# ishine/minimax-speech

Measured on AMD Instinct MI355X. Metric: 24 kHz audio-seconds generated per wall-second per node (CosyVoice2-0.5B-shaped LM + flow + DAC-VAE, end to end), higher is better.
Workload: dtype bf16

## Files before the change

### include/mmx_hip.h

```cpp
#ifndef MMX_HIP_H
#define MMX_HIP_H
#include <stdint.h>
#ifdef __cplusplus
extern "C" {
#endif

#ifndef __HIP__
typedef struct ihipStream_t* hipStream_t;
#endif

#define MMX_F32 0
#define MMX_BF16 1
#define MMX_X2 2
#define MMX_X3 3
#define MMX_X2W 0x12
#define MMX_X3W 0x13
#define MMX_H2 4
#define MMX_H2W 0x14

#define MMX_ACT_NONE 0
#define MMX_ACT_LRELU 1
#define MMX_ACT_GELU 2
#define MMX_ACT_SILU 3
#define MMX_ACT_MISH 4
#define MMX_ACT_TANH 5

int mmx_abi_version(void);

typedef struct MmxGemmParams {
    const void* A;
    const void* W;
    const float* bias;
    const float* residual;
    const float* rowmask;
    const float* alpha;
    float* out_f32;
    void* out_act;
    int64_t lda, ldw, ldr, ldo_f, ldo_a;
    int64_t a_bstride, w_bstride, r_bstride, rm_bstride, of_bstride, oa_bstride;
    int64_t row_off, row_lo, row_hi;
    int64_t out_off, out_len;
    int32_t M, N, batch;
    int32_t ntaps, cin, dil;
    int32_t bias_mod, alpha_mod, bias_per_row;
    int32_t act, act2;
    float slope;
    int32_t row_stride;
} MmxGemmParams;
int mmx_gemm_win(const MmxGemmParams* p, int dtype, hipStream_t stream);
#define MMX_TILE_128x128 1
#define MMX_TILE_128x64 2
#define MMX_TILE_64x64 3
#define MMX_TILE_32x64 4
int mmx_gemm_win_tile(const MmxGemmParams* p, int dtype, int tile, hipStream_t stream);

int mmx_rownorm(const float* x, int64_t ldx, int64_t x_bstride, int rows, int C, int batch,
                const float* gamma, const float* beta, float eps, int rms, int act,
                const float* rowmask, int64_t rm_bstride, const float* addvec, int64_t av_bstride,
                float* out_f32, int64_t ldo_f, int64_t of_bstride,
                void* out_act, int64_t ldo_a, int64_t oa_bstride, int dtype, hipStream_t stream);

int mmx_groupnorm(const float* x, int B, int T, int C, int groups, const float* gamma, const float* beta, float eps,
                  int act, const float* rowmask, void* out, int dtype, hipStream_t stream);

int mmx_act_rows(const float* x, int64_t rows, int C, int act, const float* rowmask, float* out_f32, void* out_act, int dtype,
                 hipStream_t stream);

int mmx_gather_rows(const int64_t* ids, int n, const float* table, int C, float scale, const float* rowmask,
                    float* out_f32, int64_t ldo_f, void* out_act, int64_t ldo_a, int dtype, hipStream_t stream);

int mmx_copy2d(const void* in, int in_dtype, int64_t ibs, int64_t irs, int64_t ics, int rep,
               void* out, int out_dtype, int64_t obs, int64_t ors, int64_t ocs,
               int rows, int cols, int batch, hipStream_t stream);

int mmx_est_pack(const float* x, int64_t x_bs, int x_mod, const float* mu, const float* spks, const float* cond, int B, int T, int C,
                 void* h, int64_t ldh, int dtype, hipStream_t stream);
int mmx_sinusoidal_emb(const float* t, int B, int dim, float scale, void* out, int dtype, hipStream_t stream);

int mmx_cfg_euler(float* x, const float* d_cond, const float* d_uncond, float cfg, float dt, int64_t n,
                  hipStream_t stream);

int mmx_attn_dense(const void* q, int64_t ldq, int64_t q_bs, const void* k, int64_t ldk, int64_t k_bs,
                   const void* v, int64_t ldv, int64_t v_bs, void* out, int64_t ldo, int64_t o_bs,
                   int B, int H, int D, int Tq, int Tk, float scale, const float* keymask, int64_t km_bs, int chunk,
                   const void* pos, int64_t ldp, const float* pos_u, const float* pos_v,
                   int head_stride, int q_begin, int dtype, hipStream_t stream);
int mmx_attn_flash_bf16(const void* q, int64_t ldq, int64_t q_bs, const void* k, int64_t ldk, int64_t k_bs,
                        const void* vt, int64_t ldvt, int64_t vt_bs, void* out, int64_t ldo, int64_t o_bs,
                        int B, int H, int T, float scale, const float* keymask, int64_t km_bs, int chunk, int q_begin,
                        const int32_t* klen, hipStream_t stream);
int mmx_attn_relpos_x(const float* q, int64_t ldq, int64_t q_bs, const float* k, int64_t ldk, int64_t k_bs, const float* v,
                      int64_t ldv, int64_t v_bs, const float* pos, int64_t ldp, const float* pos_u, const float* pos_v,
                      float* out, int64_t ldo, int64_t o_bs, int B, int H, int T, float scale, int chunk, const int32_t* klen,
                      hipStream_t stream);
int mmx_attn_flash_x(const float* q, int64_t ldq, int64_t q_bs, const float* k, int64_t ldk, int64_t k_bs,
                     const float* v, int64_t ldv, int64_t v_bs, float* out, int64_t ldo, int64_t o_bs,
                     int B, int H, int T, float scale, const float* keymask, int64_t km_bs, int chunk,
                     int q_begin, const int32_t* klen, hipStream_t stream);
int mmx_attn_flash_xs(const void* qk, int64_t ldqk, int64_t qk_bs, const void* vt, int64_t ldvt, int64_t vt_bs,
                      float* out, int64_t ldo, int64_t o_bs, int B, int H, int T, float scale, const float* keymask,
                      int64_t km_bs, int chunk, int q_begin, const int32_t* klen, int form, hipStream_t stream);
int mmx_attn_relpos_bf16(const void* q, int64_t ldq, int64_t q_bs, const void* k, int64_t ldk, int64_t k_bs,
                         const void* vt, int64_t ldvt, int64_t vt_bs, const void* pos, int64_t ldp,
                         const float* pos_u, const float* pos_v, void* out, int64_t ldo, int64_t o_bs,
                         int B, int H, int T, float scale, int chunk, const int32_t* klen, hipStream_t stream);

int mmx_attn_flash_fp8(const void* q, int64_t ldq, int64_t q_bs, const void* k, int64_t ldk, int64_t k_bs,
                       const void* vt, int64_t ldvt, int64_t vt_bs, void* out, int64_t ldo, int64_t o_bs,
                       int B, int H, int T, float scale, const float* keymask, int64_t km_bs, int chunk, int q_begin,
                       const int32_t* klen, hipStream_t stream);

int mmx_conv_cin1(const float* x, int64_t x_bs, int T, int C, int k, const float* w, const float* bias, float slope,
                  const float* alpha, float* out_f32, void* out_act, int batch, int dtype, hipStream_t stream);
int mmx_vae_sample(const float* ml, const float* noise, int64_t rows, int D, float* z, float* m, float* logs,
                   hipStream_t stream);
int mmx_mask_rows(void* x, int64_t rows, int C, const float* rowmask, int dtype, hipStream_t stream);
int mmx_pool_rows(const float* x, int64_t x_bs, int rows, int C, int batch, const float* mask, int64_t m_bs, void* out,
                  int64_t ldo, int dtype, hipStream_t stream);
int mmx_prefetch4(const void* p0, int64_t n0, const void* p1, int64_t n1, const void* p2, int64_t n2, const void* p3, int64_t n3,
                  void* sink, int workgroups, hipStream_t stream);
int mmx_resample_linear(const float* x, int64_t rows, int T, int T2, float* out, hipStream_t stream);

int mmx_conv_cout1_tanh(const void* act, int64_t a_bs, int T, int C, int k, const float* w, const float* bias,
                        float slope, int use_tanh, float* out, int64_t o_bs, int batch, int dtype, hipStream_t stream);

#define MMX_X_PACKED 1
#define MMX_OUT_PACKED 2
int mmx_pack_skinny(const void* w, int64_t ldw, int N, int K, const float* kscale, int interleave_half,
                    void* wp, int dtype, hipStream_t stream);
int mmx_skinny_gemm(const void* x, int x_dtype, int64_t ldx, int B, int K, int N, const void* wp,
                    const float* bias, int rs, float eps, int epi, float* out_f32, int64_t ldo_f,
                    void* out_act, int64_t ldo_a, int dtype, int flags, const float* kgamma, hipStream_t stream);

int mmx_decode_prep(const float* x, int64_t ldx, int B, int K, const float* gamma, float* h, int64_t ldh, void* xs,
                    float* ssq, int dtype, hipStream_t stream);
int mmx_skinny2(const void* xs, int B, int K, int N, const void* wp, const float* bias, const float* ssq_in, float eps,
                int epi, float* out, int64_t ldo, void* xs_out, const float* gamma_next, float* ssq_out,
                int tiles_per_wg, int ksplit, float* part, int64_t part_floats, int32_t* tickets, int dtype,
                hipStream_t stream);

int mmx_rope_kv_store(const float* qkv, int64_t ldqkv, int64_t qkv_bs, int B, int rows, int Hq, int Hkv, int D,
                      const float* inv_freq, const int32_t* pos, void* q_out, int64_t ldq, int64_t q_bs,
                      void* kc, void* vc, const int32_t* block_table, int max_pages, int page,
                      int dtype, hipStream_t stream);
int mmx_paged_attn(const void* q, int64_t ldq, int64_t q_bs, int B, int rows, int Hq, int Hkv, int D, float scale,
                   const int32_t* pos, const void* kc, const void* vc, const int32_t* block_table, int max_pages,
                   int page, void* out, int64_t ldo, int64_t o_bs, int dtype, hipStream_t stream);
#define MMX_DA_PACKED 1
#define MMX_DA_PER_HEAD 2
#define MMX_DA_SPLIT 4
#define MMX_DA_H2 8
#define MMX_DA_ONE_HEAD 16
int mmx_decode_attn(const float* qkv, int64_t ldqkv, int B, int Hq, int Hkv, int D, const float* inv_freq,
                    const float* rope_tab, const int32_t* pos, void* kc, void* vc, const int32_t* block_table, int max_pages, int page,
                    float scale, void* out, int64_t ldo, int dtype, int out_packed, hipStream_t stream);
int mmx_decode_attn_fin(const float* qkv, int64_t ldqkv, int B, int Hq, int Hkv, int D, const float* inv_freq,
                        const float* rope_tab, const int32_t* pos, const int32_t* finished, void* kc, void* vc,
                        const int32_t* block_table, int max_pages, int page, float scale, void* out, int64_t ldo, int dtype,
                        int out_packed, hipStream_t stream);
int mmx_swiglu(const float* gu, int64_t ldgu, int rows, int I, void* out, int64_t ldo, int dtype, hipStream_t stream);

int mmx_sample_step(const float* logits, int64_t ldl, int V, int B, int eos_id, int top_k, float top_p,
                    int win_size, float tau_r, uint64_t seed, int32_t* state, int32_t* out_tokens, int max_out,
                    int32_t* sampled, const int32_t* forced, const float* speech_emb, int E, float* next_x,
                    int64_t ldx, float* logp_out, hipStream_t stream);
int mmx_sample_step_tab(const float* logits, int64_t ldl, int V, int B, int eos_id, const int32_t* samp, int32_t* state,
                        int32_t* out_tokens, int max_out, int32_t* sampled, const int32_t* forced, const float* speech_emb,
                        int E, float* next_x, int64_t ldx, float* logp_out, hipStream_t stream);

typedef struct MmxEstNext {
    const void* wqkv;
    const float* n1g;
    const float* n1b;
    void* q_out;
    void* vt_out;
    int64_t q_bs, vt_bs;
    int32_t ldq, ldvt;
} MmxEstNext;
typedef struct MmxEstTailParams {
    const void* ao;
    float* x;
    const void* wo;
    const void* w1;
    const void* w2;
    const float* bo;
    const float* b1;
    const float* b2;
    const float* n3g;
    const float* n3b;
    const float* rowmask;
    void* act_out;
    int64_t ao_bs, x_bs, rm_bs, act_bs;
    int32_t ldao, act_ld, B, T;
    int32_t t_begin;
    float eps;
    MmxEstNext next;
} MmxEstTailParams;
typedef struct MmxEstResnetParams {
    const void* a_in;
    float* x;
    const void* w1;
    const void* w2;
    const void* wr;
    const float* b1;
    const float* g1;
    const float* be1;
    const float* b2;
    const float* g2;
    const float* be2;
    const float* br;
    const float* tv;
    const float* rowmask;
    int64_t a_bs, x_bs, tv_bs, rm_bs;
    int32_t lda, cin, B, T;
    int32_t t_begin;
    float eps;
    MmxEstNext next;
} MmxEstResnetParams;
int mmx_est_tail(const MmxEstTailParams* p, int dtype, int bm, int cfg, hipStream_t stream);
int mmx_est_resnet(const MmxEstResnetParams* p, int dtype, int bm, int cfg, hipStream_t stream);
typedef struct {
    const float* x;
    float* x_out;
    void* act_out;
    const void* w7;
    const void* w1;
    const float* b7;
    const float* b1;
    const float* a0;
    const float* a2;
    const float* alpha_next;
    const int32_t* lens;
    int64_t x_bs;
    int32_t B, T, C, dil;
    float slope;
} MmxDacRuParams;
int mmx_dac_ru(const MmxDacRuParams* p, int dtype, int bm, hipStream_t stream);

int mmx_logmel(const float* wave, int64_t w_bs, int L, int B, const float* gain, const int32_t* lens, const int32_t* h_lens,
               const void* basis, const void* filt, int n_fft, int hop, int bin0, int n_bins, int n_mels, float* out_cm,
               int64_t ldo, void* out_tm, int T, int dtype, hipStream_t stream);

int mmx_logmel_w(const float* wave, int64_t w_bs, int L, int B, const int32_t* lens, const int32_t* h_lens, const void* basis,
                 const void* filt, int n_fft, int hop, int bin0, int n_bins, int n_mels, float* out_cm, int64_t ldo,
                 void* out_tm, int T, int dtype, hipStream_t stream);

int mmx_s3_rope_fsmn(float* qkv, int64_t ldqkv, int64_t qkv_bs, int B, int T, int C, const float* x, int64_t x_bs, float* r,
                     int64_t r_bs, const float* wt, const float* rope_cos, const float* rope_sin, int rope_rows,
                     const int32_t* lens, hipStream_t stream);

int mmx_fsq_encode(const float* x, int64_t ldx, int64_t x_bs, int B, int T, int C, const float* W, const float* bias,
                   const int32_t* lens, int32_t* ids, int64_t ld_ids, float* pre, hipStream_t stream);

#define MMX_RESAMPLE_NOUT 1024
int mmx_resample_sinc(const float* wave, int64_t w_bs, int L, int B, const int32_t* lens, const int32_t* h_lens, int orig, int neu,
                      int width, const float* taps, const int32_t* first, const int32_t* count, int cmax, float* out,
                      int64_t o_bs, int out_cols, hipStream_t stream);

#define MMX_LOUD_PAD 0
#define MMX_LOUD_DROP 1
#define MMX_LOUD_MAX_CH 5
int mmx_kweight_blocks(const float* wave, int64_t w_bs, int L, int B, const int32_t* lens, int rate, int partial, const double* tab,
                       int seg, double* work, int cap, double* energy, int64_t e_bs, float* peak, hipStream_t stream);
int mmx_loudness_gate(const double* energy, int64_t e_bs, int cap, const float* peak, const int32_t* lens, int L, int nclips, int nch,
                      const double* G, int rate, int partial, float* lufs, int want_gain, float target_db, float max_peak, float* gain,
                      uint8_t* mask, int64_t mask_bs, hipStream_t stream);
int mmx_scale_rows(const float* x, int64_t x_bs, int L, int B, const int32_t* lens, const float* gain, int nch, float* out,
                   int64_t o_bs, hipStream_t stream);

int mmx_spec_dist(const float* x, int64_t x_bs, const float* y, int64_t y_bs, int L, int B, const int32_t* lens, const int32_t* h_lens,
                  const void* basis, const void* filt, int n_fft, int n_mels, double eps, double pow, double* work, int cap,
                  double* out, hipStream_t stream);
int mmx_wave_sums(const float* x, int64_t x_bs, const float* y, int64_t y_bs, int L, int B, const int32_t* lens, float clip, double* work,
                  int cap, double* out, hipStream_t stream);

int mmx_gate_threshold(const float* x, int64_t x_bs, int L, int B, const int32_t* lens, const int32_t* h_lens, const void* basis,
                       int n_fft, double n_std, double* work, int cap, float* thresh, int64_t t_bs, hipStream_t stream);
int mmx_gate_analyze(const float* x, int64_t x_bs, int L, int B, const int32_t* lens, const int32_t* h_lens, const void* basis, int n_fft,
                     const float* thresh, int64_t t_bs, float* spec, uint8_t* mask, int frames_cap, hipStream_t stream);
int mmx_gate_synthesize(const float* spec, const uint8_t* mask, int frames_cap, int L, int B, const int32_t* lens, const int32_t* h_lens,
                        const void* inv, const float* window, int n_fft, int n_freq, int n_time, const float* amount, float* frames,
                        float* out, int64_t o_bs, hipStream_t stream);

int mmx_stoi_select(const float* ref, int64_t r_bs, int L, int B, const int32_t* lens, const int32_t* h_lens, const float* window,
                    double* energy, uint8_t* mask, int32_t* map, int32_t* kept, int cap, hipStream_t stream);
int mmx_stoi_bands(const float* est, int64_t e_bs, const float* ref, int64_t r_bs, int L, int B, const int32_t* lens,
                   const int32_t* h_lens, const float* window, const int32_t* map, const int32_t* kept, const void* basis,
                   const void* filt, float* env, int cap, hipStream_t stream);
int mmx_stoi_score(const float* env, int cap, int B, const int32_t* kept, int extended, double* work, int wcap, double* out,
                   int32_t* frames, hipStream_t stream);

int mmx_ir_prepare(const float* ir, int64_t ir_bs, int Lir, int B, const int32_t* ir_lens, const int32_t* h_ir_lens, int Lsig,
                   const int32_t* sig_lens, const int32_t* h_sig_lens, const float* drr, int t0, const double* hann, int start_at_max,
                   float* h_out, int64_t h_bs, int32_t* p, float* s, int32_t* taps, float* drr_out, void* table, int kcap,
                   hipStream_t stream);
int mmx_fir_rows(const float* x, int64_t x_bs, int L, int B, const int32_t* lens, const int32_t* h_lens, const void* table, int kcap,
                 const int32_t* p, const float* s, const int32_t* taps, int wrap, float* out, int64_t o_bs, float* peak,
                 hipStream_t stream);
int mmx_row_absmax(const float* x, int64_t x_bs, int L, int B, const int32_t* lens, float* peak, hipStream_t stream);
int mmx_mix_rows(const float* x, int64_t x_bs, int L, int B, const int32_t* lens, const float* noise, int64_t n_bs, int Ln,
                 const int32_t* nlens, const float* lx, const float* ln, const float* snr, float* out, int64_t o_bs, hipStream_t stream);

#ifdef __cplusplus
}
#endif
#endif
```

### minimax-speech_amd/csrc/gemm.hip

```cpp
#include <algorithm>
#include "common.h"
#include "gemm.h"
#include <utility>

template <typename T> struct Frag;
template <> struct Frag<bf16_t> {
    static constexpr int CH = 8;
    static constexpr int LDS_ROW = 48;
};
template <> struct Frag<float> {
    static constexpr int CH = 4;
    static constexpr int LDS_ROW = 40;
};

template <typename T, typename TA, int NS, int BM, int BN, int WM, int WN, int NWP = 1>
__global__ __launch_bounds__(256) void gemm_win_kernel(GemmParams p) {
    constexpr int BK = 32;
    constexpr bool XS = NS > 1;
    static_assert(NWP == 1 || NWP == NS, "weight planes: as many as activation planes");
    static_assert(!XS || (sizeof(T) == 2 && sizeof(TA) == 4), "split build: bf16 weights, fp32 activations");
    static_assert(XS || sizeof(T) == sizeof(TA), "one storage type otherwise");
    constexpr int CH = Frag<T>::CH;
    constexpr int CPR = BK / CH;
    constexpr int CHA = 16 / sizeof(TA);
    constexpr int CPRA = BK / CHA;
    constexpr int LR = Frag<T>::LDS_ROW;
    constexpr int MF = BM / WM / 16, NF = BN / WN / 16;
    constexpr int A_CHUNKS = (BM * CPRA + 255) / 256, W_CHUNKS = (BN * CPR + 255) / 256;
    constexpr bool A_FULL = (BM * CPRA) % 256 == 0, W_FULL = (BN * CPR) % 256 == 0;
    constexpr bool PRECISE = sizeof(TA) == 4;

    extern __shared__ __attribute__((aligned(16))) char smem[];
    T* As = reinterpret_cast<T*>(smem);
    T* Ws = As + NS * 2 * BM * LR;

    const int tid = threadIdx.x, lane = tid & 63, wave = tid >> 6;
    const int wm = wave / WN, wn = wave % WN;
    const int g = lane >> 4, l16 = lane & 15;
    const int b = blockIdx.z;
    const int m0 = blockIdx.y * BM, n0 = blockIdx.x * BN;

    const TA* A = reinterpret_cast<const TA*>(p.A) + (long)b * p.a_bstride;
    const T* W = reinterpret_cast<const T*>(p.W) + (long)b * p.w_bstride;

    constexpr unsigned OOB = 0x80000000u;
    const auto a_rsrc = __builtin_amdgcn_make_buffer_rsrc(const_cast<TA*>(A), 0, 0x7fffffff, 0x00020000);
    const auto w_rsrc = __builtin_amdgcn_make_buffer_rsrc(const_cast<T*>(W), 0, 0x7fffffff, 0x00020000);
    unsigned a_off[A_CHUNKS];
    int a_c[A_CHUNKS], a_tap[A_CHUNKS];
    long a_srow[A_CHUNKS];
    bool a_mok[A_CHUNKS];
    const unsigned tap_jump = (unsigned)(((long)p.dil * p.lda - p.cin) * (long)sizeof(TA));
#pragma unroll
    for (int i = 0; i < A_CHUNKS; ++i) {
        const int id = tid + i * 256;
        const int r = id / CPRA, k = (id % CPRA) * CHA;
        const int m = m0 + r;
        a_tap[i] = k / p.cin;
        a_c[i] = k % p.cin;
        a_srow[i] = (long)m * p.row_stride + (long)a_tap[i] * p.dil + p.row_off;
        a_off[i] = (unsigned)((a_srow[i] * p.lda + a_c[i]) * (long)sizeof(TA));
        a_mok[i] = (m < p.M) && (A_FULL || id < BM * CPRA);
    }
    unsigned w_off[W_CHUNKS];
#pragma unroll
    for (int i = 0; i < W_CHUNKS; ++i) {
        const int id = tid + i * 256;
        const int r = id / CPR, kc = (id % CPR) * CH;
        const int n = n0 + r;
        const bool ok = (n < p.N) && (W_FULL || id < BN * CPR);
        w_off[i] = ok ? (unsigned)(((long)n * p.ldw + kc) * (long)sizeof(T)) : OOB;
    }
    constexpr int STAGES = (sizeof(T) == 2 && !XS) ? 4 : 2;
    uint4 a_reg[STAGES][A_CHUNKS], w_reg[STAGES][NWP][W_CHUNKS];
    const unsigned w_plane = (unsigned)((p.ldw / NWP) * (long)sizeof(T));
    const int K = p.ntaps * p.cin;
    const int nk = (K + BK - 1) / BK;

    auto load_tile = [&](int kt, auto slot_c) {
        constexpr int slot = decltype(slot_c)::value;
        typedef __attribute__((ext_vector_type(4))) unsigned int u32x4_t;
#pragma unroll
        for (int i = 0; i < A_CHUNKS; ++i) {
            const bool ok = a_mok[i] && (a_tap[i] < p.ntaps) && (a_srow[i] >= p.row_lo) && (a_srow[i] < p.row_hi);
            const u32x4_t v = __builtin_amdgcn_raw_buffer_load_b128(a_rsrc, ok ? a_off[i] : OOB, 0, 0);
            a_reg[slot][i] = make_uint4(v[0], v[1], v[2], v[3]);
            a_off[i] += BK * (unsigned)sizeof(TA);
            a_c[i] += BK;
            while (a_c[i] >= p.cin) {
                a_c[i] -= p.cin;
                a_tap[i]++;
                a_srow[i] += p.dil;
                a_off[i] += tap_jump;
            }
        }
#pragma unroll
        for (int i = 0; i < W_CHUNKS; ++i) {
#pragma unroll
            for (int p2 = 0; p2 < NWP; ++p2) {
                const u32x4_t v = __builtin_amdgcn_raw_buffer_load_b128(w_rsrc, (kt < nk && w_off[i] != OOB) ? w_off[i] + p2 * w_plane : OOB, 0, 0);
                w_reg[slot][p2][i] = make_uint4(v[0], v[1], v[2], v[3]);
            }
            if (w_off[i] != OOB) w_off[i] += BK * (unsigned)sizeof(T);
        }
    };
    auto store_tile = [&](int stage, auto slot_c) {
        constexpr int slot = decltype(slot_c)::value;
#pragma unroll
        for (int i = 0; i < A_CHUNKS; ++i) {
            int id = tid + i * 256;
            if (A_FULL || id < BM * CPRA) {
                if constexpr (XS) {
                    const uint4 v = a_reg[slot][i];
                    float x[4] = {__uint_as_float(v.x), __uint_as_float(v.y), __uint_as_float(v.z), __uint_as_float(v.w)};
#pragma unroll
                    for (int s2 = 0; s2 < NS; ++s2) {
                        uint2 pk;
                        pk.x = pack_bf16x2(x[0], x[1]);
                        pk.y = pack_bf16x2(x[2], x[3]);
                        *reinterpret_cast<uint2*>(As + ((s2 * 2 + stage) * BM + id / CPRA) * LR + (id % CPRA) * CHA) = pk;
                        if (s2 + 1 < NS) {
                            x[0] -= __uint_as_float(pk.x << 16); x[1] -= __uint_as_float(pk.x & 0xffff0000u);
                            x[2] -= __uint_as_float(pk.y << 16); x[3] -= __uint_as_float(pk.y & 0xffff0000u);
                        }
                    }
                } else {
                    *reinterpret_cast<uint4*>(As + (stage * BM + id / CPRA) * LR + (id % CPRA) * CHA) = a_reg[slot][i];
                }
            }
        }
#pragma unroll
        for (int i = 0; i < W_CHUNKS; ++i) {
            int id = tid + i * 256;
            if (W_FULL || id < BN * CPR) {
#pragma unroll
                for (int p2 = 0; p2 < NWP; ++p2)
                    *reinterpret_cast<uint4*>(Ws + ((p2 * 2 + stage) * BN + id / CPR) * LR + (id % CPR) * CH) = w_reg[slot][p2][i];
            }
        }
    };

    float4_t acc[MF][NF];
#pragma unroll
    for (int i = 0; i < MF; ++i)
#pragma unroll
        for (int j = 0; j < NF; ++j) acc[i][j] = float4_t{0.f, 0.f, 0.f, 0.f};

    auto compute = [&](int st) {
        const T* as = As + (st * BM + wm * (BM / WM) + l16) * LR;
        const T* ws = Ws + (st * BN + wn * (BN / WN) + l16) * LR;
        if constexpr (sizeof(T) == 2) {
            short8_t bfr[NWP][NF];
#pragma unroll
            for (int p2 = 0; p2 < NWP; ++p2)
#pragma unroll
                for (int j = 0; j < NF; ++j) bfr[p2][j] = *reinterpret_cast<const short8_t*>(ws + p2 * 2 * BN * LR + j * 16 * LR + 8 * g);
#pragma unroll
            for (int s2 = 0; s2 < NS; ++s2) {
                short8_t af[MF];
#pragma unroll
                for (int i = 0; i < MF; ++i) af[i] = *reinterpret_cast<const short8_t*>(as + s2 * 2 * BM * LR + i * 16 * LR + 8 * g);
#pragma unroll
                for (int p2 = 0; p2 < NWP; ++p2) {
                    if (s2 + p2 >= NS) continue;
#pragma unroll
                    for (int i = 0; i < MF; ++i)
#pragma unroll
                        for (int j = 0; j < NF; ++j)
                            acc[i][j] = __builtin_amdgcn_mfma_f32_16x16x32_bf16(af[i], bfr[p2][j], acc[i][j], 0, 0, 0);
                }
            }
        } else {
#pragma unroll
            for (int c = 0; c < 2; ++c) {
                float4_t af[MF], bfr[NF];
#pragma unroll
                for (int i = 0; i < MF; ++i) af[i] = *reinterpret_cast<const float4_t*>(as + i * 16 * LR + 16 * c + 4 * g);
#pragma unroll
                for (int j = 0; j < NF; ++j) bfr[j] = *reinterpret_cast<const float4_t*>(ws + j * 16 * LR + 16 * c + 4 * g);
#pragma unroll
                for (int s = 0; s < 4; ++s)
#pragma unroll
                    for (int i = 0; i < MF; ++i)
#pragma unroll
                        for (int j = 0; j < NF; ++j)
                            acc[i][j] = __builtin_amdgcn_mfma_f32_16x16x4f32(af[i][s], bfr[j][s], acc[i][j], 0, 0, 0);
            }
        }
    };
    auto for_each_slot = [&](auto&& fn) {
        [&]<int... S>(std::integer_sequence<int, S...>) { (fn(std::integral_constant<int, S>{}), ...); }
        (std::make_integer_sequence<int, STAGES>{});
    };
    for_each_slot([&](auto sc) { load_tile(decltype(sc)::value, sc); });
    int kt0 = 0;
    for (; kt0 + STAGES <= nk; kt0 += STAGES) {
        for_each_slot([&](auto sc) {
            const int kt = kt0 + decltype(sc)::value;
            store_tile(decltype(sc)::value & 1, sc);
            load_tile(kt + STAGES, sc);
            __syncthreads();
            compute(decltype(sc)::value & 1);
        });
    }
    for_each_slot([&](auto sc) {
        const int kt = kt0 + decltype(sc)::value;
        if (kt < nk) {
            store_tile(decltype(sc)::value & 1, sc);
            __syncthreads();
            compute(decltype(sc)::value & 1);
        }
    });

    __syncthreads();
    constexpr int WNC = BN / WN;
    constexpr int CW = WNC / 4;
    constexpr int LDC = WNC + 4;
    float* Cs = reinterpret_cast<float*>(smem) + wave * 16 * LDC;
    float* outf = p.out_f32 ? p.out_f32 + (long)b * p.of_bstride : nullptr;
    TA* outa = p.out_act ? reinterpret_cast<TA*>(p.out_act) + (long)b * p.oa_bstride : nullptr;
    const float* res = p.residual ? p.residual + (long)b * p.r_bstride : nullptr;
    const float* rmask = p.rowmask ? p.rowmask + (long)b * p.rm_bstride : nullptr;
    constexpr int VA = 16 / sizeof(TA);
    const bool vec_f = outf && (p.ldo_f % 4 == 0) && (p.out_off % 4 == 0) && (p.of_bstride % 4 == 0) && ((uintptr_t)p.out_f32 % 16 == 0);
    const bool vec_a = outa && (p.ldo_a % VA == 0) && (p.out_off % VA == 0) && (p.oa_bstride % VA == 0) && ((uintptr_t)p.out_act % 16 == 0) && (CW % VA == 0);
    const bool vec_r = res && (p.ldr % 4 == 0) && (p.r_bstride % 4 == 0) && ((uintptr_t)p.residual % 16 == 0);
    const int erow = lane >> 2, ecol = (lane & 3) * CW;
    auto epilogue = [&](auto act_k, auto act2_k) {
    constexpr int ACT = decltype(act_k)::value, ACT2 = decltype(act2_k)::value;
#pragma unroll
    for (int i = 0; i < MF; ++i) {
#pragma unroll
        for (int j = 0; j < NF; ++j)
#pragma unroll
            for (int r = 0; r < 4; ++r) Cs[(4 * g + r) * LDC + j * 16 + l16] = acc[i][j][r];
        __builtin_amdgcn_fence(__ATOMIC_RELEASE, "wavefront");
        __builtin_amdgcn_wave_barrier();
        float v[CW];
#pragma unroll
        for (int c = 0; c < CW; c += 4) {
            float4_t t4 = *reinterpret_cast<const float4_t*>(Cs + erow * LDC + ecol + c);
            v[c] = t4[0]; v[c + 1] = t4[1]; v[c + 2] = t4[2]; v[c + 3] = t4[3];
        }
        __builtin_amdgcn_wave_barrier();
        const int m = m0 + wm * (BM / WM) + i * 16 + erow;
        const int nb = n0 + wn * WNC + ecol;
        if (m >= p.M || nb >= p.N) continue;
        const bool full = nb + CW <= p.N;
        const float rm = rmask ? rmask[m] : 1.f;
        float rr[CW];
        if (res) {
            if (vec_r && full) {
#pragma unroll
                for (int c = 0; c < CW; c += 4) {
                    float4_t t4 = *reinterpret_cast<const float4_t*>(res + (long)m * p.ldr + nb + c);
                    rr[c] = t4[0]; rr[c + 1] = t4[1]; rr[c + 2] = t4[2]; rr[c + 3] = t4[3];
                }
            } else {
#pragma unroll
                for (int c = 0; c < CW; ++c) rr[c] = (nb + c < p.N) ? res[(long)m * p.ldr + nb + c] : 0.f;
            }
        }
        int bidx = p.bias ? (p.bias_per_row ? m : nb % p.bias_mod) : 0;
        int aidx = p.alpha ? nb % p.alpha_mod : 0;
        float w2[CW];
#pragma unroll
        for (int c = 0; c < CW; ++c) {
            float x = v[c];
            if (p.bias) {
                x += p.bias[bidx];
                if (!p.bias_per_row && ++bidx == p.bias_mod) bidx = 0;
            }
            x = act_c<ACT, PRECISE>(x, p.slope);
            if (res) x += rr[c];
            x *= rm;
            v[c] = x;
            if (outa) {
                float w = act_c<ACT2, PRECISE>(x, p.slope);
                if (p.alpha) {
                    w = snake_apply<PRECISE>(w, p.alpha[aidx]);
                    if (++aidx == p.alpha_mod) aidx = 0;
                }
                w2[c] = w;
            }
        }
        if (outf) {
            const long lin = (long)m * p.ldo_f + nb + p.out_off;
            if (vec_f && full && lin >= 0 && lin + CW <= p.out_len) {
#pragma unroll
                for (int c = 0; c < CW; c += 4)
                    *reinterpret_cast<float4_t*>(outf + lin + c) = float4_t{v[c], v[c + 1], v[c + 2], v[c + 3]};
            } else {
#pragma unroll
                for (int c = 0; c < CW; ++c)
                    if (nb + c < p.N && lin + c >= 0 && lin + c < p.out_len) outf[lin + c] = v[c];
            }
        }
        if (outa) {
            const long lin = (long)m * p.ldo_a + nb + p.out_off;
            if (vec_a && full && lin >= 0 && lin + CW <= p.out_len) {
                if constexpr (sizeof(TA) == 2) {
#pragma unroll
                    for (int c = 0; c < CW; c += 8) {
                        uint4 pk;
                        pk.x = pack_bf16x2(w2[c], w2[c + 1]);
                        pk.y = pack_bf16x2(w2[c + 2], w2[c + 3]);
                        pk.z = pack_bf16x2(w2[c + 4], w2[c + 5]);
                        pk.w = pack_bf16x2(w2[c + 6], w2[c + 7]);
                        *reinterpret_cast<uint4*>(outa + lin + c) = pk;
                    }
                } else {
#pragma unroll
                    for (int c = 0; c < CW; c += 4)
                        *reinterpret_cast<float4_t*>(outa + lin + c) = float4_t{w2[c], w2[c + 1], w2[c + 2], w2[c + 3]};
                }
            } else {
#pragma unroll
                for (int c = 0; c < CW; ++c)
                    if (nb + c < p.N && lin + c >= 0 && lin + c < p.out_len) outa[lin + c] = Cvt<TA>::from_f(w2[c]);
            }
        }
    }
    };
    using std::integral_constant;
    switch (p.act) {
        case ACT_LRELU: epilogue(integral_constant<int, ACT_LRELU>{}, integral_constant<int, ACT_NONE>{}); break;
        case ACT_GELU: epilogue(integral_constant<int, ACT_GELU>{}, integral_constant<int, ACT_NONE>{}); break;
        case ACT_SILU: epilogue(integral_constant<int, ACT_SILU>{}, integral_constant<int, ACT_NONE>{}); break;
        case ACT_MISH: epilogue(integral_constant<int, ACT_MISH>{}, integral_constant<int, ACT_NONE>{}); break;
        case ACT_TANH: epilogue(integral_constant<int, ACT_TANH>{}, integral_constant<int, ACT_NONE>{}); break;
        default:
            if (p.act2 == ACT_MISH) epilogue(integral_constant<int, ACT_NONE>{}, integral_constant<int, ACT_MISH>{});
            else epilogue(integral_constant<int, ACT_NONE>{}, integral_constant<int, ACT_NONE>{});
    }
}

template <typename T, typename TA, int NS, int BM, int BN, int WM, int WN, int NWP = 1>
static int launch_cfg(const GemmParams& p, hipStream_t s) {
    dim3 grid((p.N + BN - 1) / BN, (p.M + BM - 1) / BM, p.batch);
    size_t lds = (size_t)2 * (NS * BM + NWP * BN) * Frag<T>::LDS_ROW * sizeof(T);
    const size_t lds_epi = (size_t)4 * 16 * (BN / WN + 4) * sizeof(float);
    if (lds_epi > lds) lds = lds_epi;
    MMX_LDS_OPT_IN((gemm_win_kernel<T, TA, NS, BM, BN, WM, WN, NWP>), lds);
    hipLaunchKernelGGL((gemm_win_kernel<T, TA, NS, BM, BN, WM, WN, NWP>), grid, dim3(256), lds, s, p);
    MMX_LAUNCH_CHECK();
    return MMX_OK;
}

template <typename T, typename TA, int NS, int NWP = 1>
static int launch_T(const GemmParams& p, hipStream_t s, int force_tile) {
    constexpr int CH = Frag<T>::CH;
    constexpr int CHA = 16 / sizeof(TA);
    MMX_CHECK_ARG(p.A && p.W && p.M > 0 && p.N > 0 && p.batch > 0 && p.ntaps >= 1);
    MMX_CHECK_ARG(p.cin % CH == 0 && p.lda % CHA == 0 && p.ldw % CH == 0);
    MMX_CHECK_ARG(p.a_bstride % CHA == 0 && p.w_bstride % CH == 0);
    MMX_CHECK_ARG(p.ldw % NWP == 0 && (p.ldw / NWP) % CH == 0 && p.ldw / NWP >= ((p.ntaps * p.cin + 31) / 32) * 32);
    MMX_CHECK_ARG(p.bias_mod > 0 && p.alpha_mod > 0 && p.row_stride >= 1);
    MMX_CHECK_ARG(((uintptr_t)p.A % 16) == 0 && ((uintptr_t)p.W % 16) == 0);
    MMX_CHECK_ARG(p.out_f32 || p.out_act);
    const long a_rows = std::min<long>(p.row_hi, (long)(p.M - 1) * p.row_stride + (long)(p.ntaps - 1) * p.dil + p.row_off + 1);
    MMX_CHECK_ARG((double)a_rows * (double)p.lda * sizeof(TA) < 2147483000.0 &&
                  (double)p.N * (double)p.ldw * sizeof(T) < 2147483000.0);
    MMX_CHECK_ARG(p.act2 == ACT_NONE || (p.act2 == ACT_MISH && p.act == ACT_NONE));
    auto blocks = [&](int bm, int bn) { return (long)((p.M + bm - 1) / bm) * ((p.N + bn - 1) / bn) * p.batch; };
    if constexpr (NWP > 1) {
        if (force_tile != 0 && force_tile != MMX_TILE_64x64 && force_tile != MMX_TILE_32x64) return MMX_EARG;
        if (force_tile != MMX_TILE_32x64 && (force_tile == MMX_TILE_64x64 || blocks(64, 64) >= 64 || p.M > 32))
            return launch_cfg<T, TA, NS, 64, 64, 2, 2, NWP>(p, s);
        return launch_cfg<T, TA, NS, 32, 64, 1, 4, NWP>(p, s);
    }
    switch (force_tile) {
        case 0: break;
        case MMX_TILE_128x128: return launch_cfg<T, TA, NS, 128, 128, 2, 2>(p, s);
        case MMX_TILE_128x64: return launch_cfg<T, TA, NS, 128, 64, 4, 1>(p, s);
        case MMX_TILE_64x64: return launch_cfg<T, TA, NS, 64, 64, 2, 2>(p, s);
        case MMX_TILE_32x64: return launch_cfg<T, TA, NS, 32, 64, 1, 4>(p, s);
        default: return MMX_EARG;
    }
    const long b128 = blocks(128, 128);
    if (p.N > 64 && (b128 >= 1024 || (p.ntaps * p.cin >= 1024 && b128 >= 512))) return launch_cfg<T, TA, NS, 128, 128, 2, 2>(p, s);
    if (p.N <= 64 && blocks(128, 64) >= 512) return launch_cfg<T, TA, NS, 128, 64, 4, 1>(p, s);
    if (blocks(64, 64) >= 64 || p.M > 32) return launch_cfg<T, TA, NS, 64, 64, 2, 2>(p, s);
    return launch_cfg<T, TA, NS, 32, 64, 1, 4>(p, s);
}

extern "C" int mmx_gemm_win_tile(const GemmParams* p, int dtype, int tile, hipStream_t stream) {
    MMX_CHECK_ARG(p != nullptr);
    if (dtype == MMX_BF16) return launch_T<bf16_t, bf16_t, 1>(*p, stream, tile);
    if (dtype == MMX_F32) return launch_T<float, float, 1>(*p, stream, tile);
    if (dtype == MMX_X2) return launch_T<bf16_t, float, 2>(*p, stream, tile);
    if (dtype == MMX_X3) return launch_T<bf16_t, float, 3>(*p, stream, tile);
    if (dtype == MMX_X2W) return launch_T<bf16_t, float, 2, 2>(*p, stream, tile);
    if (dtype == MMX_X3W) return launch_T<bf16_t, float, 3, 3>(*p, stream, tile);
    return MMX_EARG;
}
extern "C" int mmx_gemm_win(const GemmParams* p, int dtype, hipStream_t stream) {
    return mmx_gemm_win_tile(p, dtype, 0, stream);
}
```

### minimax-speech_amd/mmx/_lib.py

```python
import ctypes as C
import os

import torch

F32, BF16 = 0, 1
X2, X3 = 2, 3
X2W, X3W = 0x12, 0x13
H2, H2W = 4, 0x14
DA_PACKED, DA_PER_HEAD, DA_SPLIT, DA_H2, DA_ONE_HEAD = 1, 2, 4, 8, 16
ACT = {"none": 0, "lrelu": 1, "gelu": 2, "silu": 3, "mish": 4, "tanh": 5}
TORCH_DT = {F32: torch.float32, BF16: torch.bfloat16, X2: torch.float32, X3: torch.float32, X2W: torch.float32, X3W: torch.float32}
WEIGHT_DT = {F32: torch.float32, BF16: torch.bfloat16, X2: torch.bfloat16, X3: torch.bfloat16, X2W: torch.bfloat16, X3W: torch.bfloat16}
ESIZE = {F32: 4, BF16: 2, X2: 4, X3: 4}
WPLANES = {X2W: 2, X3W: 3}
DTYPE_NAMES = {"f32": F32, "bf16": BF16, "x": X2, "x2": X2, "x3": X3}


def is_split(dtype):
    return dtype in (X2, X3, X2W, X3W)

_HERE = os.path.dirname(os.path.abspath(__file__))
LIB_PATH = os.environ.get("MMX_LIB") or os.path.join(os.path.dirname(_HERE), "lib", "libmmx_hip.so")

SYMBOLS = [
    "mmx_abi_version", "mmx_gemm_win", "mmx_gemm_win_tile", "mmx_rownorm", "mmx_groupnorm", "mmx_act_rows", "mmx_gather_rows", "mmx_copy2d", "mmx_est_pack",
    "mmx_sinusoidal_emb", "mmx_cfg_euler", "mmx_attn_dense", "mmx_attn_flash_bf16", "mmx_attn_flash_fp8", "mmx_attn_relpos_bf16", "mmx_attn_relpos_x", "mmx_attn_flash_x", "mmx_attn_flash_xs", "mmx_conv_cout1_tanh", "mmx_conv_cin1", "mmx_vae_sample", "mmx_resample_linear", "mmx_prefetch4", "mmx_mask_rows",
    "mmx_est_tail", "mmx_est_resnet", "mmx_dac_ru", "mmx_pack_skinny", "mmx_skinny_gemm", "mmx_skinny2", "mmx_decode_prep", "mmx_rope_kv_store", "mmx_paged_attn", "mmx_decode_attn", "mmx_decode_attn_fin", "mmx_swiglu", "mmx_sample_step",
    "mmx_sample_step_tab", "mmx_logmel", "mmx_pool_rows", "mmx_logmel_w", "mmx_s3_rope_fsmn", "mmx_fsq_encode", "mmx_resample_sinc", "mmx_kweight_blocks", "mmx_loudness_gate", "mmx_scale_rows",
    "mmx_spec_dist", "mmx_wave_sums", "mmx_gate_threshold", "mmx_gate_analyze", "mmx_gate_synthesize",
    "mmx_stoi_select", "mmx_stoi_bands", "mmx_stoi_score",
    "mmx_ir_prepare", "mmx_fir_rows", "mmx_row_absmax", "mmx_mix_rows",
]


class GemmParams(C.Structure):
    _fields_ = [
        ("A", C.c_void_p), ("W", C.c_void_p), ("bias", C.c_void_p), ("residual", C.c_void_p),
        ("rowmask", C.c_void_p), ("alpha", C.c_void_p), ("out_f32", C.c_void_p), ("out_act", C.c_void_p),
        ("lda", C.c_int64), ("ldw", C.c_int64), ("ldr", C.c_int64), ("ldo_f", C.c_int64), ("ldo_a", C.c_int64),
        ("a_bstride", C.c_int64), ("w_bstride", C.c_int64), ("r_bstride", C.c_int64), ("rm_bstride", C.c_int64),
        ("of_bstride", C.c_int64), ("oa_bstride", C.c_int64),
        ("row_off", C.c_int64), ("row_lo", C.c_int64), ("row_hi", C.c_int64),
        ("out_off", C.c_int64), ("out_len", C.c_int64),
        ("M", C.c_int32), ("N", C.c_int32), ("batch", C.c_int32),
        ("ntaps", C.c_int32), ("cin", C.c_int32), ("dil", C.c_int32),
        ("bias_mod", C.c_int32), ("alpha_mod", C.c_int32), ("bias_per_row", C.c_int32),
        ("act", C.c_int32), ("act2", C.c_int32), ("slope", C.c_float), ("row_stride", C.c_int32),
    ]


class EstNext(C.Structure):
    _fields_ = [("wqkv", C.c_void_p), ("n1g", C.c_void_p), ("n1b", C.c_void_p), ("q_out", C.c_void_p), ("vt_out", C.c_void_p),
                ("q_bs", C.c_int64), ("vt_bs", C.c_int64), ("ldq", C.c_int32), ("ldvt", C.c_int32)]


class EstTailParams(C.Structure):
    _fields_ = [(k, C.c_void_p) for k in ("ao", "x", "wo", "w1", "w2", "bo", "b1", "b2", "n3g", "n3b", "rowmask", "act_out")] + \
               [(k, C.c_int64) for k in ("ao_bs", "x_bs", "rm_bs", "act_bs")] + \
               [(k, C.c_int32) for k in ("ldao", "act_ld", "B", "T", "t_begin")] + [("eps", C.c_float), ("next", EstNext)]


class EstResnetParams(C.Structure):
    _fields_ = [(k, C.c_void_p) for k in ("a_in", "x", "w1", "w2", "wr", "b1", "g1", "be1", "b2", "g2", "be2", "br", "tv", "rowmask")] + \
               [(k, C.c_int64) for k in ("a_bs", "x_bs", "tv_bs", "rm_bs")] + \
               [(k, C.c_int32) for k in ("lda", "cin", "B", "T", "t_begin")] + [("eps", C.c_float), ("next", EstNext)]


class DacRuParams(C.Structure):
    _fields_ = [(k, C.c_void_p) for k in ("x", "x_out", "act_out", "w7", "w1", "b7", "b1", "a0", "a2", "alpha_next", "lens")] + \
               [("x_bs", C.c_int64)] + [(k, C.c_int32) for k in ("B", "T", "C", "dil")] + [("slope", C.c_float)]


def fill_struct(st, **kw):
    for k, v in kw.items():
        if v is not None and hasattr(v, "data_ptr"):
            assert v.is_cuda
            v = v.data_ptr()
        setattr(st, k, v)
    return st


ABI_VERSION = 10
_lib = None


class MmxError(RuntimeError):
    pass


def load():
    global _lib
    if _lib is None:
        if not os.path.exists(LIB_PATH):
            raise MmxError(f"{LIB_PATH} not found: build it with `make -C minimax-speech_amd/csrc` "
                           "(or __graft_entry__.build()); the hot path has no CPU fallback")
        lib = C.CDLL(LIB_PATH)
        for s in SYMBOLS:
            getattr(lib, s).restype = C.c_int
        if lib.mmx_abi_version() != ABI_VERSION:
            raise MmxError(f"{LIB_PATH} has ABI version {lib.mmx_abi_version()}, this package binds version {ABI_VERSION}: "
                           "rebuild it (`make -C minimax-speech_amd/csrc`)")
        _lib = lib
    return _lib


def _p(t):
    if t is None:
        return None
    if isinstance(t, int):
        return C.c_void_p(t)
    assert t.is_cuda, "libmmx_hip works on device memory only (no CPU fallback)"
    return C.c_void_p(t.data_ptr())


def stream():
    return C.c_void_p(torch.cuda.current_stream().cuda_stream)


def check(rc, what):
    if rc != 0:
        raise MmxError(f"{what} failed with code {rc}" + (" (argument/shape error)" if rc == -1 else ""))


def dt_of(t):
    return BF16 if t.dtype == torch.bfloat16 else F32


def i64(x):
    return C.c_int64(int(x))


def gemm_params(**kw):
    p = GemmParams()
    p.bias_mod = 1
    p.alpha_mod = 1
    p.ntaps = 1
    p.dil = 1
    p.batch = 1
    p.row_lo = 0
    p.out_len = 1 << 62
    p.slope = 0.1
    p.row_stride = 1
    for k, v in kw.items():
        if k in ("A", "W", "bias", "residual", "rowmask", "alpha", "out_f32", "out_act"):
            v = None if v is None else (v if isinstance(v, int) else v.data_ptr())
        setattr(p, k, v)
    return p


TILES = {"auto": 0, "128x128": 1, "128x64": 2, "64x64": 3, "32x64": 4}


def gemm_win(p, dtype, tile=0):
    if tile:
        check(load().mmx_gemm_win_tile(C.byref(p), C.c_int(dtype), C.c_int(tile), stream()), "mmx_gemm_win_tile")
    else:
        check(load().mmx_gemm_win(C.byref(p), C.c_int(dtype), stream()), "mmx_gemm_win")
```

Before: 569.6.

## Add deep-K 512-thread GEMM tiles for large DAC conv7 split-precision GEMMs

Generalizes the windowed GEMM kernel so thread count, K-depth per LDS stage (BK=64) and pipeline stage count are template parameters. It adds two deep-K configurations (128x128 and 128x256 with 8 waves) and selects the 128x256 one automatically for split-build GEMMs with K>=4096, N a multiple of 256 and enough workgroups, which matches the DAC block-1 conv7 shapes. The goal is more reuse per LDS load and fewer barriers per K for these large convolutions. In exchange it uses more LDS and registers per workgroup, which may lower occupancy. The ragged-K tail handling is also new code.

```diff
diff --git a/include/mmx_hip.h b/include/mmx_hip.h
--- a/include/mmx_hip.h
+++ b/include/mmx_hip.h
@@ -52,6 +52,8 @@
 #define MMX_TILE_128x64 2
 #define MMX_TILE_64x64 3
 #define MMX_TILE_32x64 4
+#define MMX_TILE_DEEP_128x128 5
+#define MMX_TILE_DEEP_128x256 6
 int mmx_gemm_win_tile(const MmxGemmParams* p, int dtype, int tile, hipStream_t stream);
 
 int mmx_rownorm(const float* x, int64_t ldx, int64_t x_bstride, int rows, int C, int batch,
diff --git a/minimax-speech_amd/csrc/gemm.hip b/minimax-speech_amd/csrc/gemm.hip
--- a/minimax-speech_amd/csrc/gemm.hip
+++ b/minimax-speech_amd/csrc/gemm.hip
@@ -13,10 +13,12 @@
     static constexpr int LDS_ROW = 40;
 };
 
-template <typename T, typename TA, int NS, int BM, int BN, int WM, int WN, int NWP = 1>
-__global__ __launch_bounds__(256) void gemm_win_kernel(GemmParams p) {
-    constexpr int BK = 32;
+template <typename T, typename TA, int NS, int BM, int BN, int WM, int WN, int NWP = 1, int KS = 1, int STG = 0>
+__global__ __launch_bounds__(WM * WN * 64) void gemm_win_kernel(GemmParams p) {
+    constexpr int NT = WM * WN * 64;
+    constexpr int BK = 32 * KS;
     constexpr bool XS = NS > 1;
+    static_assert(KS == 1 || (KS == 2 && XS && NWP == 1), "deep-K form: split build, one weight plane");
     static_assert(NWP == 1 || NWP == NS, "weight planes: as many as activation planes");
     static_assert(!XS || (sizeof(T) == 2 && sizeof(TA) == 4), "split build: bf16 weights, fp32 activations");
     static_assert(XS || sizeof(T) == sizeof(TA), "one storage type otherwise");
@@ -24,10 +26,10 @@
     constexpr int CPR = BK / CH;
     constexpr int CHA = 16 / sizeof(TA);
     constexpr int CPRA = BK / CHA;
-    constexpr int LR = Frag<T>::LDS_ROW;
+    constexpr int LR = KS == 1 ? Frag<T>::LDS_ROW : BK + 16;
     constexpr int MF = BM / WM / 16, NF = BN / WN / 16;
-    constexpr int A_CHUNKS = (BM * CPRA + 255) / 256, W_CHUNKS = (BN * CPR + 255) / 256;
-    constexpr bool A_FULL = (BM * CPRA) % 256 == 0, W_FULL = (BN * CPR) % 256 == 0;
+    constexpr int A_CHUNKS = (BM * CPRA + NT - 1) / NT, W_CHUNKS = (BN * CPR + NT - 1) / NT;
+    constexpr bool A_FULL = (BM * CPRA) % NT == 0, W_FULL = (BN * CPR) % NT == 0;
     constexpr bool PRECISE = sizeof(TA) == 4;
 
     extern __shared__ __attribute__((aligned(16))) char smem[];
@@ -53,7 +55,7 @@
     const unsigned tap_jump = (unsigned)(((long)p.dil * p.lda - p.cin) * (long)sizeof(TA));
 #pragma unroll
     for (int i = 0; i < A_CHUNKS; ++i) {
-        const int id = tid + i * 256;
+        const int id = tid + i * NT;
         const int r = id / CPRA, k = (id % CPRA) * CHA;
         const int m = m0 + r;
         a_tap[i] = k / p.cin;
@@ -65,17 +67,18 @@
     unsigned w_off[W_CHUNKS];
 #pragma unroll
     for (int i = 0; i < W_CHUNKS; ++i) {
-        const int id = tid + i * 256;
+        const int id = tid + i * NT;
         const int r = id / CPR, kc = (id % CPR) * CH;
         const int n = n0 + r;
         const bool ok = (n < p.N) && (W_FULL || id < BN * CPR);
         w_off[i] = ok ? (unsigned)(((long)n * p.ldw + kc) * (long)sizeof(T)) : OOB;
     }
-    constexpr int STAGES = (sizeof(T) == 2 && !XS) ? 4 : 2;
+    constexpr int STAGES = STG ? STG : (sizeof(T) == 2 && !XS) ? 4 : 2;
     uint4 a_reg[STAGES][A_CHUNKS], w_reg[STAGES][NWP][W_CHUNKS];
     const unsigned w_plane = (unsigned)((p.ldw / NWP) * (long)sizeof(T));
     const int K = p.ntaps * p.cin;
-    const int nk = (K + BK - 1) / BK;
+    const int nk32 = (K + 31) / 32;
+    const int nk = (nk32 + KS - 1) / KS;
 
     auto load_tile = [&](int kt, auto slot_c) {
         constexpr int slot = decltype(slot_c)::value;
@@ -98,7 +101,9 @@
         for (int i = 0; i < W_CHUNKS; ++i) {
 #pragma unroll
             for (int p2 = 0; p2 < NWP; ++p2) {
-                const u32x4_t v = __builtin_amdgcn_raw_buffer_load_b128(w_rsrc, (kt < nk && w_off[i] != OOB) ? w_off[i] + p2 * w_plane : OOB, 0, 0);
+                bool ok = kt < nk && w_off[i] != OOB;
+                if constexpr (KS > 1) ok = ok && kt * BK + ((tid + i * NT) % CPR) * CH < nk32 * 32;
+                const u32x4_t v = __builtin_amdgcn_raw_buffer_load_b128(w_rsrc, ok ? w_off[i] + p2 * w_plane : OOB, 0, 0);
                 w_reg[slot][p2][i] = make_uint4(v[0], v[1], v[2], v[3]);
             }
             if (w_off[i] != OOB) w_off[i] += BK * (unsigned)sizeof(T);
@@ -108,7 +113,7 @@
         constexpr int slot = decltype(slot_c)::value;
 #pragma unroll
         for (int i = 0; i < A_CHUNKS; ++i) {
-            int id = tid + i * 256;
+            int id = tid + i * NT;
             if (A_FULL || id < BM * CPRA) {
                 if constexpr (XS) {
                     const uint4 v = a_reg[slot][i];
@@ -131,7 +136,7 @@
         }
 #pragma unroll
         for (int i = 0; i < W_CHUNKS; ++i) {
-            int id = tid + i * 256;
+            int id = tid + i * NT;
             if (W_FULL || id < BN * CPR) {
 #pragma unroll
                 for (int p2 = 0; p2 < NWP; ++p2)
@@ -146,9 +151,14 @@
 #pragma unroll
         for (int j = 0; j < NF; ++j) acc[i][j] = float4_t{0.f, 0.f, 0.f, 0.f};
 
-    auto compute = [&](int st) {
-        const T* as = As + (st * BM + wm * (BM / WM) + l16) * LR;
-        const T* ws = Ws + (st * BN + wn * (BN / WN) + l16) * LR;
+    auto compute = [&](int st, int steps) {
+        const T* as0 = As + (st * BM + wm * (BM / WM) + l16) * LR;
+        const T* ws0 = Ws + (st * BN + wn * (BN / WN) + l16) * LR;
+#pragma unroll
+        for (int ks = 0; ks < KS; ++ks) {
+        if (ks >= steps) break;
+        const T* as = as0 + ks * 32;
+        const T* ws = ws0 + ks * 32;
         if constexpr (sizeof(T) == 2) {
             short8_t bfr[NWP][NF];
 #pragma unroll
@@ -186,6 +196,7 @@
                         for (int j = 0; j < NF; ++j)
                             acc[i][j] = __builtin_amdgcn_mfma_f32_16x16x4f32(af[i][s], bfr[j][s], acc[i][j], 0, 0, 0);
             }
+        }
         }
     };
     auto for_each_slot = [&](auto&& fn) {
@@ -193,22 +204,26 @@
         (std::make_integer_sequence<int, STAGES>{});
     };
     for_each_slot([&](auto sc) { load_tile(decltype(sc)::value, sc); });
+    auto lds_stage = [](int kt0, int slot) { return (STAGES % 2 == 0) ? (slot & 1) : ((kt0 + slot) & 1); };
+    const int nkf = nk32 / KS;
     int kt0 = 0;
-    for (; kt0 + STAGES <= nk; kt0 += STAGES) {
+    for (; kt0 + STAGES <= nkf; kt0 += STAGES) {
         for_each_slot([&](auto sc) {
             const int kt = kt0 + decltype(sc)::value;
-            store_tile(decltype(sc)::value & 1, sc);
+            const int st = lds_stage(kt0, decltype(sc)::value);
+            store_tile(st, sc);
             load_tile(kt + STAGES, sc);
             __syncthreads();
-            compute(decltype(sc)::value & 1);
+            compute(st, KS);
         });
     }
     for_each_slot([&](auto sc) {
         const int kt = kt0 + decltype(sc)::value;
         if (kt < nk) {
-            store_tile(decltype(sc)::value & 1, sc);
+            const int st = lds_stage(kt0, decltype(sc)::value);
+            store_tile(st, sc);
             __syncthreads();
-            compute(decltype(sc)::value & 1);
+            compute(st, KS == 1 ? 1 : nk32 - kt * KS);
         }
     });
 
@@ -335,17 +350,46 @@
     }
 }
 
-template <typename T, typename TA, int NS, int BM, int BN, int WM, int WN, int NWP = 1>
+template <typename T, typename TA, int NS, int BM, int BN, int WM, int WN, int NWP = 1, int KS = 1, int STG = 0>
 static int launch_cfg(const GemmParams& p, hipStream_t s) {
     dim3 grid((p.N + BN - 1) / BN, (p.M + BM - 1) / BM, p.batch);
-    size_t lds = (size_t)2 * (NS * BM + NWP * BN) * Frag<T>::LDS_ROW * sizeof(T);
-    const size_t lds_epi = (size_t)4 * 16 * (BN / WN + 4) * sizeof(float);
+    constexpr int LR = KS == 1 ? Frag<T>::LDS_ROW : 32 * KS + 16;
+    size_t lds = (size_t)2 * (NS * BM + NWP * BN) * LR * sizeof(T);
+    static_assert((size_t)2 * (NS * BM + NWP * BN) * LR * sizeof(T) <= 160 * 1024, "operand tiles: at most the CU's 160 KB of LDS");
+    const size_t lds_epi = (size_t)WM * WN * 16 * (BN / WN + 4) * sizeof(float);
     if (lds_epi > lds) lds = lds_epi;
-    MMX_LDS_OPT_IN((gemm_win_kernel<T, TA, NS, BM, BN, WM, WN, NWP>), lds);
-    hipLaunchKernelGGL((gemm_win_kernel<T, TA, NS, BM, BN, WM, WN, NWP>), grid, dim3(256), lds, s, p);
+    MMX_LDS_OPT_IN((gemm_win_kernel<T, TA, NS, BM, BN, WM, WN, NWP, KS, STG>), lds);
+    hipLaunchKernelGGL((gemm_win_kernel<T, TA, NS, BM, BN, WM, WN, NWP, KS, STG>), grid, dim3(WM * WN * 64), lds, s, p);
     MMX_LAUNCH_CHECK();
     return MMX_OK;
 }
+
+constexpr int gemm_tile_select(int ns, int nwp, long M, long N, long K, long batch) {
+    auto blocks = [&](int bm, int bn) { return ((M + bm - 1) / bm) * ((N + bn - 1) / bn) * batch; };
+    if (nwp > 1) return (blocks(64, 64) >= 64 || M > 32) ? MMX_TILE_64x64 : MMX_TILE_32x64;
+    if (ns == 2 && N % 256 == 0 && K >= 4096 && blocks(128, 256) >= 250) return MMX_TILE_DEEP_128x256;
+    const long b128 = blocks(128, 128);
+    if (N > 64 && (b128 >= 1024 || (K >= 1024 && b128 >= 512))) return MMX_TILE_128x128;
+    if (N <= 64 && blocks(128, 64) >= 512) return MMX_TILE_128x64;
+    if (blocks(64, 64) >= 64 || M > 32) return MMX_TILE_64x64;
+    return MMX_TILE_32x64;
+}
+static_assert(gemm_tile_select(2, 1, 4460, 768, 5376, 5) == MMX_TILE_DEEP_128x256, "DAC block 1 conv7, largest flow group");
+static_assert(gemm_tile_select(2, 1, 1690, 768, 5376, 6) == MMX_TILE_DEEP_128x256, "DAC block 1 conv7, smallest measured grid");
+static_assert(gemm_tile_select(2, 1, 900, 768, 5376, 4) == MMX_TILE_64x64, "DAC block 1 conv7, 96 deep workgroups: not measured, as before");
+static_assert(gemm_tile_select(2, 1, 4460, 768, 768, 5) == MMX_TILE_128x128, "DAC block 1 conv1");
+static_assert(gemm_tile_select(2, 1, 17840, 384, 2688, 5) == MMX_TILE_128x128, "DAC block 2 conv7");
+static_assert(gemm_tile_select(2, 1, 17840, 384, 384, 5) == MMX_TILE_128x128, "DAC block 2 conv1");
+static_assert(gemm_tile_select(2, 1, 893, 3840, 3072, 5) == MMX_TILE_128x128, "DAC block 1 transposed conv");
+static_assert(gemm_tile_select(3, 1, 1600, 9728, 896, 1) == MMX_TILE_64x64, "prompt pass gate / up");
+static_assert(gemm_tile_select(3, 1, 1600, 896, 4864, 1) == MMX_TILE_64x64, "prompt pass down");
+static_assert(gemm_tile_select(3, 1, 1600, 1152, 896, 1) == MMX_TILE_64x64, "prompt pass q / k / v");
+static_assert(gemm_tile_select(3, 1, 1600, 896, 896, 1) == MMX_TILE_64x64, "prompt pass o");
+static_assert(gemm_tile_select(2, 1, 896, 256, 768, 10) == MMX_TILE_64x64, "flow ResNet conv, 10 sequences");
+static_assert(gemm_tile_select(2, 1, 2000, 1024, 256, 1) == MMX_TILE_64x64, "flow GELU projection");
+static_assert(gemm_tile_select(2, 1, 2000, 256, 1024, 1) == MMX_TILE_64x64, "flow feed-forward out");
+static_assert(gemm_tile_select(2, 1, 512, 1024, 256, 16) == MMX_TILE_64x64, "flow, 16 sequences: 256 128-tiles");
+static_assert(gemm_tile_select(2, 1, 10, 3584, 1024, 1) == MMX_TILE_32x64, "flow time embedding");
 
 template <typename T, typename TA, int NS, int NWP = 1>
 static int launch_T(const GemmParams& p, hipStream_t s, int force_tile) {
@@ -362,26 +406,24 @@
     MMX_CHECK_ARG((double)a_rows * (double)p.lda * sizeof(TA) < 2147483000.0 &&
                   (double)p.N * (double)p.ldw * sizeof(T) < 2147483000.0);
     MMX_CHECK_ARG(p.act2 == ACT_NONE || (p.act2 == ACT_MISH && p.act == ACT_NONE));
-    auto blocks = [&](int bm, int bn) { return (long)((p.M + bm - 1) / bm) * ((p.N + bn - 1) / bn) * p.batch; };
+    const int tile = force_tile ? force_tile : gemm_tile_select(NS, NWP, p.M, p.N, (long)p.ntaps * p.cin, p.batch);
     if constexpr (NWP > 1) {
-        if (force_tile != 0 && force_tile != MMX_TILE_64x64 && force_tile != MMX_TILE_32x64) return MMX_EARG;
-        if (force_tile != MMX_TILE_32x64 && (force_tile == MMX_TILE_64x64 || blocks(64, 64) >= 64 || p.M > 32))
-            return launch_cfg<T, TA, NS, 64, 64, 2, 2, NWP>(p, s);
-        return launch_cfg<T, TA, NS, 32, 64, 1, 4, NWP>(p, s);
-    }
-    switch (force_tile) {
-        case 0: break;
-        case MMX_TILE_128x128: return launch_cfg<T, TA, NS, 128, 128, 2, 2>(p, s);
-        case MMX_TILE_128x64: return launch_cfg<T, TA, NS, 128, 64, 4, 1>(p, s);
-        case MMX_TILE_64x64: return launch_cfg<T, TA, NS, 64, 64, 2, 2>(p, s);
-        case MMX_TILE_32x64: return launch_cfg<T, TA, NS, 32, 64, 1, 4>(p, s);
-        default: return MMX_EARG;
-    }
-    const long b128 = blocks(128, 128);
-    if (p.N > 64 && (b128 >= 1024 || (p.ntaps * p.cin >= 1024 && b128 >= 512))) return launch_cfg<T, TA, NS, 128, 128, 2, 2>(p, s);
-    if (p.N <= 64 && blocks(128, 64) >= 512) return launch_cfg<T, TA, NS, 128, 64, 4, 1>(p, s);
-    if (blocks(64, 64) >= 64 || p.M > 32) return launch_cfg<T, TA, NS, 64, 64, 2, 2>(p, s);
-    return launch_cfg<T, TA, NS, 32, 64, 1, 4>(p, s);
+        if (tile == MMX_TILE_64x64) return launch_cfg<T, TA, NS, 64, 64, 2, 2, NWP>(p, s);
+        if (tile == MMX_TILE_32x64) return launch_cfg<T, TA, NS, 32, 64, 1, 4, NWP>(p, s);
+        return MMX_EARG;
+    } else {
+        if constexpr (NS > 1)
+            if (tile == MMX_TILE_DEEP_128x128) return launch_cfg<T, TA, NS, 128, 128, 2, 4, 1, 2, 3>(p, s);
+        if constexpr (NS == 2)
+            if (tile == MMX_TILE_DEEP_128x256) return launch_cfg<T, TA, NS, 128, 256, 2, 4, 1, 2, 2>(p, s);
+        switch (tile) {
+            case MMX_TILE_128x128: return launch_cfg<T, TA, NS, 128, 128, 2, 2>(p, s);
+            case MMX_TILE_128x64: return launch_cfg<T, TA, NS, 128, 64, 4, 1>(p, s);
+            case MMX_TILE_64x64: return launch_cfg<T, TA, NS, 64, 64, 2, 2>(p, s);
+            case MMX_TILE_32x64: return launch_cfg<T, TA, NS, 32, 64, 1, 4>(p, s);
+            default: return MMX_EARG;
+        }
+    }
 }
 
 extern "C" int mmx_gemm_win_tile(const GemmParams* p, int dtype, int tile, hipStream_t stream) {
diff --git a/minimax-speech_amd/mmx/_lib.py b/minimax-speech_amd/mmx/_lib.py
--- a/minimax-speech_amd/mmx/_lib.py
+++ b/minimax-speech_amd/mmx/_lib.py
@@ -148,7 +148,7 @@
     return p
 
 
-TILES = {"auto": 0, "128x128": 1, "128x64": 2, "64x64": 3, "32x64": 4}
+TILES = {"auto": 0, "128x128": 1, "128x64": 2, "64x64": 3, "32x64": 4, "deep128x128": 5, "deep128x256": 6}
 
 
 def gemm_win(p, dtype, tile=0):
```

Measured after the change: 570.7, median of 6. Within noise of the previous version (+0.2%).
